# AlexGr5/StereoVision

Measured on AMD Instinct MI355X. Metric: disparity frames/sec + HBM GB/s, 1920x1080 D=128 win=9, 1/2/4/8 GPU, higher is better.
Workload: dtype u8

## Files before the change

### stereovision_amd/csrc/sv_match.hip

```cpp
#include "sv_internal.h"
#include "sv_xcd.h"

#include <algorithm>
#include <cstdlib>
#include <vector>
#include <cstdio>
#include <type_traits>

namespace sv {
namespace {

constexpr int COST_SAD4 = 4;

__host__ __device__ __forceinline__ int seg_width(int lpg, int dpl, int sm = 4) { return (sm * lpg + dpl - 1) / dpl * dpl; }
__host__ __device__ __forceinline__ int wave_cols(int lpg, int dpl, int sm = 4) { return (64 / lpg) * seg_width(lpg, dpl, sm); }
int seg_mult(int kind, int r) {
    static const int sm4 = [] {
        const char* e = std::getenv("SV_SAD4_SEG");
        const int v = e ? std::atoi(e) : 0;
        return v >= 1 && v <= 8 ? v : 0;
    }();
    if (kind != COST_SAD4) return 4;
    if (sm4) return sm4;
    return (2 * r - 2 + 3) / 4 <= 2 ? 4 : 2;
// ... 133 lines not shown
            }
#pragma unroll
            for (int q = 0; q < 4; ++q) {
                const int pos = j <= 2 ? j - q : (j >= 2 * r + 1 ? (3 - q) + (j - 2 * r - 1) : -1);
                const bool in = j <= 2 ? (j >= q) : (j >= 2 * r + 1 && j <= 2 * r + q);
                w[NC + q] |= in ? v << (8 * pos) : 0u;
            }
        }
        put<COST, ND>(dst, w);
    } else {
        uint32_t w[5] = {0u, 0u, 0u, 0u, 0u};
        uint32_t sq = 0;
        for (int j = 0; j < a.win; ++j) {
            const int yy = clampi(y - a.r + j, 0, a.H - 1);
            const uint32_t v = img[(size_t)yy * a.pitch + cc];
            sq += v * v;
            const uint32_t sh = v << (8 * (j & 3));
            const int q = j >> 2;
            w[0] |= q == 0 ? sh : 0u;
            w[1] |= q == 1 ? sh : 0u;
            w[2] |= q == 2 ? sh : 0u;
            w[3] |= q == 3 ? sh : 0u;
        }
        if constexpr (COST == COST_SSD) w[ND] = sq;
        const uint32_t o[8] = {w[0], w[1], w[2], w[3], w[4], 0u, 0u, 0u};
        put<COST, ND>(dst, o);
    }
}

__device__ __forceinline__ void transpose4(uint32_t a, uint32_t b, uint32_t c, uint32_t d, uint32_t (&o)[4]) {
    const uint32_t t0 = __builtin_amdgcn_perm(b, a, 0x05010400u);
    const uint32_t t1 = __builtin_amdgcn_perm(b, a, 0x07030602u);
    const uint32_t t2 = __builtin_amdgcn_perm(d, c, 0x05010400u);
    const uint32_t t3 = __builtin_amdgcn_perm(d, c, 0x07030602u);
    o[0] = __builtin_amdgcn_perm(t2, t0, 0x05040100u);
    o[1] = __builtin_amdgcn_perm(t2, t0, 0x07060302u);
    o[2] = __builtin_amdgcn_perm(t3, t1, 0x05040100u);
    o[3] = __builtin_amdgcn_perm(t3, t1, 0x07060302u);
}

template <int R>
__device__ __forceinline__ void sad4_group_words(const uint32_t (&rw)[2 * R + 4],
                                                 uint32_t (&w)[PackCfg<COST_SAD4, R>::NW][4]) {
    constexpr int NC = PackCfg<COST_SAD4, R>::NW - 4, NCR = 2 * R - 2;
#pragma unroll
    for (int m = 0; m < NC; ++m) {
        uint32_t d[4];
#pragma unroll
        for (int t = 0; t < 4; ++t) d[t] = 4 * m + t < NCR ? rw[3 + 4 * m + t] : 0u;
        transpose4(d[0], d[1], d[2], d[3], w[m]);
    }
#pragma unroll
    for (int q = 0; q < 4; ++q) {
        uint32_t d[3];
        int n = 0;
#pragma unroll
        for (int j = q; j <= 2; ++j) d[n++] = rw[j];
#pragma unroll
        for (int j = 2 * R + 1; j <= 2 * R + q; ++j) d[n++] = rw[j];
        transpose4(d[0], d[1], d[2], 0u, w[NC + q]);
    }
}

template <int COST, int ND>
__device__ __forceinline__ void build_group(const MatchParams& a, const uint8_t* img, int cg, int y,
                                            uint32_t (&w)[PackCfg<COST, ND>::NW][4]) {
    const int r = COST == COST_SAD4 ? ND : a.r;
    auto row = [&](int j) -> uint32_t {
        const int yy = clampi(y - r + j, 0, a.H - 1);
        return *reinterpret_cast<const uint32_t*>(img + (size_t)yy * a.pitch + cg);
    };
    if constexpr (COST == COST_SAD4) {
        uint32_t rw[2 * ND + 4];
#pragma unroll
        for (int j = 0; j < 2 * ND + 4; ++j) rw[j] = row(j);
        sad4_group_words<ND>(rw, w);
        return;
    }
    const int nsh = a.win;
#pragma unroll
    for (int q = 0; q < ND; ++q) {
        uint32_t d[4];
#pragma unroll
        for (int t = 0; t < 4; ++t) d[t] = (4 * q + t < nsh) ? row(4 * q + t) : 0u;
        transpose4(d[0], d[1], d[2], d[3], w[q]);
    }
    if constexpr (COST == COST_SSD) {
#pragma unroll
        for (int k = 0; k < 4; ++k) {
            uint32_t sq = 0u;
#pragma unroll
            for (int q = 0; q < ND; ++q) sq = __builtin_amdgcn_udot4(w[q][k], w[q][k], sq, false);
            w[ND][k] = sq;
        }
    }
}

__device__ __forceinline__ int rslot(int i, int c0, int dpl) { return i + (i + c0) / dpl; }

template <int COST, int ND, int DPL>
__device__ __forceinline__ void build_all_packs(const MatchParams& a, int y, int cL0, int NL, int cR0,
                                                int NRlog, int c0, PackOut<COST, ND> Lp,
                                                PackOut<COST, ND> Rp, int lane) {
    constexpr int NW = PackCfg<COST, ND>::NW;
    bool aligned = ((reinterpret_cast<uintptr_t>(a.L) | reinterpret_cast<uintptr_t>(a.R) |
                     (uintptr_t)a.pitch) & 3u) == 0;
    if constexpr (COST == COST_HOG) aligned = false;
    if (!aligned) {
        for (int i = lane; i < NL; i += 64) build_pack<COST, ND>(a, a.L, a.HL, cL0 + i, y, Lp + i);
        for (int i = lane; i < NRlog; i += 64)
            build_pack<COST, ND>(a, a.R, a.HR, cR0 + i, y, Rp + rslot(i, c0, DPL));
        return;
    }
    if constexpr (COST != COST_HOG) {
    const int aL = cL0 & ~3, aR = cR0 & ~3;
    const int gL = (cL0 + NL - aL + 3) >> 2, gR = (cR0 + NRlog - aR + 3) >> 2;
    for (int gi = lane; gi < gL + gR; gi += 64) {
        const bool right = gi >= gL;
        const int cg = right ? aR + 4 * (gi - gL) : aL + 4 * gi;
        const int cfirst = right ? cR0 : cL0, n = right ? NRlog : NL;
        const uint8_t* img = right ? a.R : a.L;
        const PackOut<COST, ND> base = right ? Rp : Lp;
        if (cg >= 0 && cg + 4 <= a.W) {
            uint32_t w[NW][4];
            build_group<COST, ND>(a, img, cg, y, w);
#pragma unroll
            for (int k = 0; k < 4; ++k) {
                const int idx = cg + k - cfirst;
                if (idx < 0 || idx >= n) continue;
                uint32_t v[8];
#pragma unroll
                for (int i = 0; i < 8; ++i) v[i] = i < NW ? w[i < NW ? i : 0][k] : 0u;
                put<COST, ND>(base + (right ? rslot(idx, c0, DPL) : idx), v);
            }
        } else {
#pragma unroll
            for (int k = 0; k < 4; ++k) {
                const int idx = cg + k - cfirst;
                if (idx < 0 || idx >= n) continue;
                build_pack<COST, ND>(a, img, nullptr, cg + k, y, base + (right ? rslot(idx, c0, DPL) : idx));
            }
        }
    }
    }
}

template <int R, int MF, int DPL>
__device__ __forceinline__ void build_ring_packs(const MatchParams& a, int y, int cL0, int NL, int cR0,
                                                 int NRlog, int c0, PackOut<COST_SAD4, R> Lp,
                                                 PackOut<COST_SAD4, R> Rp, int lane) {
    constexpr int NW = PackCfg<COST_SAD4, R>::NW, NRW = 2 * R + 4;
    const bool aligned = ((reinterpret_cast<uintptr_t>(a.L) | reinterpret_cast<uintptr_t>(a.R) |
                           (uintptr_t)a.pitch) & 3u) == 0;
    if (!aligned) {
        build_all_packs<COST_SAD4, R, DPL>(a, y, cL0, NL, cR0, NRlog, c0, Lp, Rp, lane);
        return;
    }
    const int aL = cL0 & ~3, aR = cR0 & ~3;
    const int gL = (cL0 + NL - aL + 3) >> 2, gR = (cR0 + NRlog - aR + 3) >> 2;
    const int G = gL + gR;
    uint32_t roff[NRW];
#pragma unroll
    for (int j = 0; j < NRW; ++j) roff[j] = (uint32_t)clampi(y - R + j, 0, a.H - 1) * (uint32_t)a.pitch;
    for (int g0 = 0; g0 < G; g0 += 64 * MF) {
        uint32_t rw[MF][NRW];
#pragma unroll
        for (int m = 0; m < MF; ++m) {
            const int gi = g0 + lane + 64 * m;
            const bool right = gi >= gL;
            const int cg = right ? aR + 4 * (gi - gL) : aL + 4 * gi;
            const bool in = gi < G && cg >= 0 && cg + 4 <= a.W;
            const uint8_t* img = (right ? a.R : a.L) + (in ? cg : 0);
#pragma unroll
            for (int j = 0; j < NRW; ++j) rw[m][j] = *reinterpret_cast<const uint32_t*>(img + roff[j]);
        }
#pragma unroll
        for (int m = 0; m < MF; ++m) {
            const int gi = g0 + lane + 64 * m;
            if (gi >= G) continue;
            const bool right = gi >= gL;
            const int cg = right ? aR + 4 * (gi - gL) : aL + 4 * gi;
            const int cfirst = right ? cR0 : cL0, n = right ? NRlog : NL;
            const PackOut<COST_SAD4, R> base = right ? Rp : Lp;
            if (cg >= 0 && cg + 4 <= a.W) {
                uint32_t w[NW][4];
                sad4_group_words<R>(rw[m], w);
#pragma unroll
                for (int k = 0; k < 4; ++k) {
                    const int idx = cg + k - cfirst;
                    if (idx < 0 || idx >= n) continue;
                    uint32_t v[8];
#pragma unroll
                    for (int i = 0; i < 8; ++i) v[i] = i < NW ? w[i < NW ? i : 0][k] : 0u;
                    put<COST_SAD4, R>(base + (right ? rslot(idx, c0, DPL) : idx), v);
                }
            } else {
#pragma unroll
                for (int k = 0; k < 4; ++k) {
                    const int idx = cg + k - cfirst;
                    if (idx < 0 || idx >= n) continue;
                    build_pack<COST_SAD4, R>(a, right ? a.R : a.L, nullptr, cg + k, y,
                                             base + (right ? rslot(idx, c0, DPL) : idx));
                }
            }
        }
    }
}

template <int COST, int ND, int DPL>
__device__ __forceinline__ void match_chunk(
    const int cut, const int dbits, PackPtr<COST, ND> rnb, PackPtr<COST, ND> rob, PackPtr<COST, ND> lnb,
    PackPtr<COST, ND> lob,
    Pk<PackCfg<COST, ND>::NW> (&rn)[DPL], Pk<PackCfg<COST, ND>::NW> (&ro)[DPL],
    uint32_t (&h)[DPL][PackCfg<COST, ND>::ROWS], const uint32_t (&mk)[DPL],
    uint32_t (&bk)[PackCfg<COST, ND>::ROWS][DPL]) {
    constexpr int NW = PackCfg<COST, ND>::NW;
    constexpr int ROWS = PackCfg<COST, ND>::ROWS;
    constexpr bool RUN = COST != COST_HOG;
    constexpr bool HI = hi_keys(COST, ND);
#pragma unroll
    for (int u = 0; u < DPL; ++u) {
        rn[u] = ld<COST, ND>(rnb + u);
        const Pk<NW> L = ld<COST, ND>(lnb + u);
        Pk<NW> LO;
        if constexpr (RUN) {
            ro[u] = ld<COST, ND>(rob + (u + (u >= cut ? 1 : 0)));
            LO = ld<COST, ND>(lob + u);
        }
#pragma unroll
        for (int k = 0; k < DPL; ++k) {
            const int sk = (u - k + DPL) % DPL;
            if constexpr (HI) {
                constexpr int NC = PackCfg<COST, ND>::NC;
                uint32_t cn = 0u, co = 0u;
#pragma unroll
                for (int i = 0; i < NC; ++i) {
                    cn = __builtin_amdgcn_sad_hi_u8(L.w[i], rn[sk].w[i], cn);
                    co = __builtin_amdgcn_sad_hi_u8(LO.w[i], ro[sk].w[i], co);
                }
                const uint32_t nch = co - cn;
#pragma unroll
                for (int q = 0; q < ROWS; ++q) {
                    const uint32_t m = __builtin_amdgcn_sad_hi_u8(LO.w[NC + q], ro[sk].w[NC + q], nch);
                    h[k][q] = __builtin_amdgcn_sad_hi_u8(L.w[NC + q], rn[sk].w[NC + q], h[k][q]) - m;
                }
                continue;
            }
            uint32_t vn[ROWS];
            ccol<COST, ND, NW>(L, rn[sk], vn);
            if constexpr (RUN) {
                uint32_t vo[ROWS];
                ccol<COST, ND, NW>(LO, ro[sk], vo);
#pragma unroll
                for (int q = 0; q < ROWS; ++q) h[k][q] = shl_add(vn[q] - vo[q], 1 << dbits, h[k][q]);
            } else {
                h[k][0] = (vn[0] << dbits) | mk[k];
            }
        }
#pragma unroll
        for (int q = 0; q < ROWS; ++q) {
            uint32_t b = 0xFFFFFFFFu;
#pragma unroll
            for (int k = 0; k < DPL; ++k) b = min(b, h[k][q]);
            bk[q][u] = b;
        }
        __builtin_amdgcn_sched_barrier(0);
    }
}

template <int LPG, int N>
__device__ __forceinline__ void reduce_batch(uint32_t* v) {
#define SV_ROR_STEP(CTRL)                                                                     \
    _Pragma("unroll") for (int i = 0; i < N; ++i)                                             \
        v[i] = min(v[i], (uint32_t)__builtin_amdgcn_update_dpp(0u, (int)v[i], CTRL, 0xF, 0xF, false));
    SV_ROR_STEP(0x121)
    SV_ROR_STEP(0x122)
    SV_ROR_STEP(0x124)
    SV_ROR_STEP(0x128)
#undef SV_ROR_STEP
    if constexpr (LPG >= 32) {
#pragma unroll
        for (int i = 0; i < N; ++i)
            v[i] = min(v[i], (uint32_t)__builtin_amdgcn_update_dpp(-1, (int)v[i], 0x142, 0xA, 0xF, false));
    }
    if constexpr (LPG == 64) {
#pragma unroll
        for (int i = 0; i < N; ++i)
            v[i] = min(v[i], (uint32_t)__builtin_amdgcn_update_dpp(-1, (int)v[i], 0x143, 0xC, 0xF, false));
    }
}

__device__ __forceinline__ void reduce_scatter16(uint32_t (&v)[16], int l) {
#define SV_RS_STEP(HALF, BIT, CTRL)                                                            \
    {                                                                                          \
        const bool hi = (l & (BIT)) != 0;                                                      \
        _Pragma("unroll") for (int k = 0; k < (HALF); ++k) {                                   \
            const uint32_t send = hi ? v[k] : v[k + (HALF)];                                   \
            const uint32_t keep = hi ? v[k + (HALF)] : v[k];                                   \
            v[k] = min(keep, (uint32_t)__builtin_amdgcn_update_dpp(0u, (int)send, CTRL, 0xF, 0xF, false)); \
        }                                                                                      \
    }
    SV_RS_STEP(8, 8, 0x140)
    SV_RS_STEP(4, 4, 0x141)
    SV_RS_STEP(2, 2, 0x1B)
    SV_RS_STEP(1, 1, 0xB1)
#undef SV_RS_STEP
}

__device__ __forceinline__ void reduce_scatter16_bm(uint32_t (&v)[16], int l) {
#define SV_BM_PAIR(A, B, CTRL, M0, M1)                                                          \
    "v_min_u32_dpp %" #A ", %" #A ", %" #A " " CTRL " row_mask:0xf bank_mask:" M0 "\n\t"      \
    "v_min_u32_dpp %" #A ", %" #B ", %" #B " " CTRL " row_mask:0xf bank_mask:" M1 "\n\t"
    asm volatile("s_nop 1\n\t"
                 SV_BM_PAIR(0, 8, "row_mirror", "0x3", "0xc") SV_BM_PAIR(1, 9, "row_mirror", "0x3", "0xc")
                 SV_BM_PAIR(2, 10, "row_mirror", "0x3", "0xc") SV_BM_PAIR(3, 11, "row_mirror", "0x3", "0xc")
                 SV_BM_PAIR(4, 12, "row_mirror", "0x3", "0xc") SV_BM_PAIR(5, 13, "row_mirror", "0x3", "0xc")
                 SV_BM_PAIR(6, 14, "row_mirror", "0x3", "0xc") SV_BM_PAIR(7, 15, "row_mirror", "0x3", "0xc")
                 : "+v"(v[0]), "+v"(v[1]), "+v"(v[2]), "+v"(v[3]), "+v"(v[4]), "+v"(v[5]), "+v"(v[6]), "+v"(v[7])
                 : "v"(v[8]), "v"(v[9]), "v"(v[10]), "v"(v[11]), "v"(v[12]), "v"(v[13]), "v"(v[14]), "v"(v[15]));
    asm volatile("s_nop 1\n\t"
                 SV_BM_PAIR(0, 4, "row_half_mirror", "0x5", "0xa") SV_BM_PAIR(1, 5, "row_half_mirror", "0x5", "0xa")
                 SV_BM_PAIR(2, 6, "row_half_mirror", "0x5", "0xa") SV_BM_PAIR(3, 7, "row_half_mirror", "0x5", "0xa")
                 : "+v"(v[0]), "+v"(v[1]), "+v"(v[2]), "+v"(v[3])
                 : "v"(v[4]), "v"(v[5]), "v"(v[6]), "v"(v[7]));
#undef SV_BM_PAIR
#define SV_RS_STEP(HALF, BIT, CTRL)                                                            \
    {                                                                                          \
// ... 148 lines not shown
    const PackPtr<COST, ND> rn0 = Rp + rslot(iN, c0, DPL);
    const PackPtr<COST, ND> ro0 = Rp + rslot(iR0, c0, DPL);
    const PackPtr<COST, ND> ln0 = Lp + (iL0 + W2);
    const PackPtr<COST, ND> lo0 = Lp + iL0;
    const int T = (S - 1 + DPL - 1) / DPL * DPL;

    for (int t0 = 0, c = 0; t0 < T; t0 += DPL, ++c) {
        match_chunk<COST, ND, DPL>(cut, dbits, rn0 + c * (DPL + 1), ro0 + c * (DPL + 1), ln0 + t0, lo0 + t0, rn,
                                   ro, h, mk, bk);
        if constexpr (ROWS * DPL == 16 || ROWS * DPL == 32) {
            if (LPG == 16) {
#pragma unroll
                for (int half = 0; half < ROWS * DPL / 16; ++half) {
                    uint32_t v[16];
#pragma unroll
                    for (int i = 0; i < 16; ++i) v[i] = bk[(16 * half + i) / DPL][i % DPL];
                    reduce_scatter16(v, l);
                    const int q = (16 * half) / DPL + l / DPL, e = t0 + l % DPL + 1, x = xs + e;
                    if (e < S && x < a.X1 && y + q < a.row1)
                        a.out[(size_t)(y + q) * a.opitch + x] = (int16_t)(((int)(v[0] & dmask) + a.minD) * 16);
                }
                continue;
            }
        }
        if constexpr (ROWS * DPL == 8) {
            uint32_t v[8];
#pragma unroll
            for (int i = 0; i < 8; ++i) v[i] = bk[i / DPL][i % DPL];
            reduce_scatter8_bm(v, lane & 15);
            uint32_t key = v[0];
            if (LPG >= 32) {
                const auto p = __builtin_amdgcn_permlane16_swap(key, key, false, false);
                key = min(p[0], p[1]);
            }
            if (LPG == 64) {
                const auto p = __builtin_amdgcn_permlane32_swap(key, key, false, false);
                key = min(p[0], p[1]);
            }
            const int i = (l >> 1) & 7, q = i / DPL, e = t0 + i % DPL + 1, x = xs + e;
            if (l < 16 && (l & 1) == 0 && e < S && x < a.X1 && y + q < a.row1)
                a.out[(size_t)(y + q) * a.opitch + x] = (int16_t)(((int)(key & dmask) + a.minD) * 16);
            continue;
        }
        const int e = t0 + j + 1;
        const int x = xs + e;
        const bool emit = j >= 0 && j < DPL && e < S && x < a.X1;
        if (LPG == 16) reduce_batch<16, ROWS * DPL>(&bk[0][0]);
        else if (LPG == 32) reduce_batch<32, ROWS * DPL>(&bk[0][0]);
        else reduce_batch<64, ROWS * DPL>(&bk[0][0]);
#pragma unroll
        for (int q = 0; q < ROWS; ++q) {
            uint32_t v = bk[q][0];
#pragma unroll
            for (int u = 1; u < DPL; ++u) v = (j == u) ? bk[q][u] : v;
            if (emit && y + q < a.row1)
                a.out[(size_t)(y + q) * a.opitch + x] = (int16_t)(((int)(v & dmask) + a.minD) * 16);
        }
    }
}

constexpr int RG_DPL = 4;

typedef unsigned short u16x2 __attribute__((ext_vector_type(2)));
__device__ __forceinline__ uint32_t pk_add16(uint32_t a, uint32_t b) {
    return __builtin_bit_cast(uint32_t, __builtin_bit_cast(u16x2, a) + __builtin_bit_cast(u16x2, b));
}
__device__ __forceinline__ uint32_t pk_sub16(uint32_t a, uint32_t b) {
    return __builtin_bit_cast(uint32_t, __builtin_bit_cast(u16x2, a) - __builtin_bit_cast(u16x2, b));
}


typedef uint32_t lds_u32x4 __attribute__((ext_vector_type(4), may_alias));
constexpr int RING_SCRATCH_BYTES = 8 * 64 * 4;

template <int R, int LPGT, bool DEFER, bool KEYS, bool SSD = false, bool LDSMIN = false>
__global__ __launch_bounds__(64, 2) void k_match_ring(MatchParams a) {
    using P = PackCfg<COST_SAD4, R>;
    constexpr int NW = P::NW, NC = P::NC, W2 = 2 * R + 1;
    static_assert(!LDSMIN || (LPGT == 32 && R <= 5), "the LDS fold is laid out for two 32-lane groups of 32-bit keys");
    constexpr bool PK = R >= 6;
    static_assert(P::SPLIT && (P::CW == 3) == PK, "ring kind expects split packs (20 B for r 2..3, 24 B for r 4..5, 28 B for r 6..7)");
    extern __shared__ __attribute__((aligned(16))) uint4 smem[];
    int bx, by, bz;
    xcd_tile(a.xcd_map != 0, bx, by, bz);
    if (bz) {
        a.L += bz * a.fs_in;
        a.R += bz * a.fs_in;
        a.out += bz * a.fs_out;
        if constexpr (KEYS) a.keys += bz * a.fs_out;
    }
    const int lane = threadIdx.x;
    constexpr int LPG = LPGT;
    const int S = a.segm;
    const int WC = (64 / LPG) * S;
    constexpr bool SADU = PK || R <= 5;
    constexpr int M = SADU ? W2 + 1 : W2;
    constexpr int U = M % 4 == 0 ? M : M % 2 == 0 ? 2 * M : 4 * M;
    constexpr int NCH = U / 4;
    const int Tn = (S + 2 * R + 3) & ~3;
    const int nit = (Tn + U - 1) / U;
    const int e0 = (nit * U - Tn) >> 2;
    const int NL = WC - S + Tn + 1;
    const int NRlog = WC - S + Tn + 4 * LPG;
    constexpr int c0 = 1;
    const int NRphys = NRlog + (NRlog + c0) / RG_DPL + 1;
    uint4* wbase = smem + (LDSMIN ? RING_SCRATCH_BYTES / 16 : 0);
    typename P::CT* cbase = reinterpret_cast<typename P::CT*>(wbase + (size_t)(NL + NRphys));
    const PackOut<COST_SAD4, R> Lw{wbase, cbase};
    const PackOut<COST_SAD4, R> Rw{wbase + NL, cbase + NL};
    const PackPtr<COST_SAD4, R> Lp{Lw.x, Lw.c};
    const PackPtr<COST_SAD4, R> Rp{Rw.x, Rw.c};

    const int y = a.row0 + by * 4;
    const int yc = min(y, a.row1 - 1);
    const int xw = a.X0 + bx * WC;
    const int cL0 = xw - R;
    const int cR0 = cL0 - a.minD - (4 * LPG - 1);
    build_ring_packs<R, 3, RG_DPL>(a, yc, cL0, NL, cR0, NRlog, c0, Lw, Rw, lane);

    if (!KEYS && bx == 0) {
        const int16_t inv = (int16_t)((a.minD - 1) * 16);
#pragma unroll
        for (int q = 0; q < 4; ++q) {
            if (y + q >= a.row1) break;
            int16_t* orow = a.out + (size_t)(y + q) * a.opitch;
            for (int x = lane; x < a.X0; x += 64) orow[x] = inv;
            for (int x = a.X1 + lane; x < a.W; x += 64) orow[x] = inv;
        }
    }
    __syncthreads();
    if (y >= a.row1) return;

    const int g = lane / LPG;
    const int l = lane & (LPG - 1);
    const int xs = xw + g * S;
    const int dl = PK ? min(4 * l, a.D - 4) : 4 * l;
    const int iR0 = g * S + 4 * (LPG - 1) - dl + 3;
    constexpr int RQ = PK ? 2 : 4;
    uint32_t h[RG_DPL][RQ], lab[RG_DPL];
#pragma unroll
    for (int k = 0; k < RG_DPL; ++k) {
        const int idx = 4 * l + k;
        const uint32_t base = PK ? 0u : idx < a.D ? (uint32_t)idx : (SSD ? a.pad_key : 0x8000u << 16) | (uint32_t)idx;
        lab[k] = (uint32_t)idx;
#pragma unroll
        for (int q = 0; q < RQ; ++q) h[k][q] = base;
    }
    uint32_t ring[M][RG_DPL][RQ];
#pragma unroll
    for (int s = 0; s < M; ++s)
#pragma unroll
        for (int k = 0; k < RG_DPL; ++k)
#pragma unroll
            for (int q = 0; q < RQ; ++q) ring[s][k][q] = 0u;
    Pk<NW> rn[RG_DPL];
#pragma unroll
    for (int s = 1; s < RG_DPL; ++s) rn[RG_DPL - s] = ld<COST_SAD4, R, true>(Rp + rslot(iR0 - s, c0, RG_DPL));
    PackPtr<COST_SAD4, R> rb = Rp + (rslot(iR0, c0, RG_DPL) - e0 * (RG_DPL + 1));
    PackPtr<COST_SAD4, R> lb = Lp + (g * S - 4 * e0);
    constexpr bool LPF = !(R == 5 && SADU);
    Pk<NW> Lnext = ld<COST_SAD4, R, true>(lb + 4 * e0);
    const int jq = (lane >> 2) & 3, ju = (lane >> 1) & 1;
    constexpr bool join2 = LPG >= 32;
    int pofs = 0;
    if (join2 && !LDSMIN) {
        const auto p = __builtin_amdgcn_permlane16_swap((uint32_t)lane, (uint32_t)lane + 64u, false, false);
        pofs = (max(p[0], p[1]) < 64u) ? 0 : 2;
    }
    const int eq = LDSMIN ? lane >> 4 : jq;
    const int exs = LDSMIN ? xw + ((lane >> 2) & 1) * S : xs;
    const int eb = (LDSMIN ? ((lane >> 3) & 1) + 2 * (lane & 1) : ju + pofs) - 2 * R;
    constexpr int OB = KEYS ? 4 : 2;
    const int ooff = OB * ((y + eq) * a.opitch + exs + eb);
    const auto orsrc = KEYS ? __builtin_amdgcn_make_buffer_rsrc(a.keys, 0, 0x7FFFFFFF, 0x00020000)
                            : __builtin_amdgcn_make_buffer_rsrc(a.out, 0, 0x7FFFFFFF, 0x00020000);
    const int emax = (LDSMIN ? (lane & 2) == 0 && y + eq < a.row1
                             : (l & 1) == 0 && l < (join2 ? 32 : 16) && y + jq < a.row1)
                         ? max(0, min(S, a.X1 - exs)) : 0;

    auto emit_key = [&](uint32_t key, int tt) {
        const int off = (unsigned)(tt + eb) < (unsigned)emax ? ooff + OB * tt : (int)0x80000000u;
        if constexpr (KEYS) __builtin_amdgcn_raw_buffer_store_b32(key, orsrc, off, 0, 0);
        else __builtin_amdgcn_raw_buffer_store_b16(
            (uint16_t)(((int)(key & (SSD ? (1u << a.dbits) - 1u : 0xFFFFu)) + a.minD) * 16), orsrc, off, 0, 0);
    };
    auto join_pairs = [&](uint32_t kA_, uint32_t kB_) {
        auto p = __builtin_amdgcn_permlane16_swap(kA_, kB_, false, false);
        uint32_t key = min(p[0], p[1]);
        if (LPG == 64) {
            p = __builtin_amdgcn_permlane32_swap(key, key, false, false);
            key = min(p[0], p[1]);
        }
        return key;
    };
    auto join_rows = [&](uint32_t key) {
        if (LPG >= 32) {
            const auto p = __builtin_amdgcn_permlane16_swap(key, key, false, false);
            key = min(p[0], p[1]);
        }
        if (LPG == 64) {
            const auto p = __builtin_amdgcn_permlane32_swap(key, key, false, false);
            key = min(p[0], p[1]);
        }
        return key;
    };
    uint32_t dv[8], kA = 0xFFFFFFFFu;
    int tprev = -(1 << 24);
#pragma unroll
    for (int i = 0; i < 8; ++i) dv[i] = 0xFFFFFFFFu;
    [[maybe_unused]] uint32_t* const scr = reinterpret_cast<uint32_t*>(smem);
    [[maybe_unused]] const uint32_t scr_m0 = __builtin_amdgcn_readfirstlane(
        (uint32_t)(uintptr_t)(__attribute__((address_space(3))) uint32_t*)scr);
    [[maybe_unused]] const lds_u32x4* const sra = reinterpret_cast<const lds_u32x4*>(scr + 8 * lane + 4 * ((lane >> 3) & 1));
    [[maybe_unused]] const lds_u32x4* const srb = reinterpret_cast<const lds_u32x4*>(scr + 8 * lane + 4 * (1 - ((lane >> 3) & 1)));
    auto lds_fold = [&](const lds_u32x4& p, const lds_u32x4& s) {
        uint32_t m = min(min(p.x, p.y), p.z);
        m = min(min(m, p.w), s.x);
        m = min(min(m, s.y), s.z);
        m = min(m, s.w);
        m = min(m, (uint32_t)__builtin_amdgcn_update_dpp(0u, (int)m, 0xB1, 0xF, 0xF, false));
        return min(m, (uint32_t)__builtin_amdgcn_update_dpp(0u, (int)m, 0x4E, 0xF, 0xF, false));
    };
    [[maybe_unused]] const bool pairB = (lane & 1) != 0;

    for (int it = 0, t0 = -4 * e0; it < nit; ++it) {
#pragma unroll
        for (int ch = 0; ch < NCH; ++ch, t0 += 4) {
            if (t0 < 0) continue;
            uint32_t bk[4][2];
#pragma unroll
            for (int u = 0; u < 4; ++u) {
                const int slot = (4 * ch + u) % M, oslot = (4 * ch + u + 1) % M;
                rn[u] = ld<COST_SAD4, R, true>(rb + (ch * (RG_DPL + 1) + u));
                const Pk<NW> Lc = LPF ? Lnext : ld<COST_SAD4, R, true>(lb + (4 * ch + u));
                if constexpr (LPF) Lnext = ld<COST_SAD4, R, true>(lb + (4 * ch + u + 1));
                lds_u32x4 fa{}, fb{};
                if constexpr (LDSMIN) {
                    if ((u & 1) == 0) { fa = *sra; fb = *srb; }
                }
                uint32_t sqL[4];
                if constexpr (SSD) {
                    uint32_t sc = 0u;
#pragma unroll
                    for (int i = 0; i < NC; ++i) sc = __builtin_amdgcn_udot4(Lc.w[i], Lc.w[i], sc, false);
#pragma unroll
                    for (int q = 0; q < 4; ++q)
                        sqL[q] = __builtin_amdgcn_udot4(Lc.w[NC + q], Lc.w[NC + q], sc, false) << a.dbits;
                }
                if constexpr (!SADU) {
#pragma unroll
                    for (int k = 0; k < RG_DPL; ++k)
#pragma unroll
                        for (int q = 0; q < RQ; ++q)
                            h[k][q] = PK ? pk_sub16(h[k][q], ring[slot][k][q]) : h[k][q] - ring[slot][k][q];
                }
#pragma unroll
                for (int kk = 0; kk < RG_DPL; ++kk) {
                    const int k = RG_DPL - 1 - kk;
                    const Pk<NW>& Rk = rn[(u - k) & 3];
                    if constexpr (PK) {
                        uint32_t cn = 0u;
#pragma unroll
                        for (int i = 0; i < NC; ++i) cn = __builtin_amdgcn_sad_u8(Lc.w[i], Rk.w[i], cn);
                        cn |= cn << 16;
#pragma unroll
                        for (int j = 0; j < 2; ++j) {
                            const uint32_t c = __builtin_amdgcn_sad_hi_u8(
                                Lc.w[NC + 2 * j + 1], Rk.w[NC + 2 * j + 1],
                                __builtin_amdgcn_sad_u8(Lc.w[NC + 2 * j], Rk.w[NC + 2 * j], cn));
                            if constexpr (SADU) sad_u32_acc(h[k][j], ring[oslot][k][j], c);
                            else h[k][j] = pk_add16(h[k][j], c);
                            ring[slot][k][j] = c;
                        }
                    } else if constexpr (SSD) {
                        uint32_t cn = 0u, sr = 0u;
#pragma unroll
                        for (int i = 0; i < NC; ++i) {
                            cn = __builtin_amdgcn_udot4(Lc.w[i], Rk.w[i], cn, false);
                            sr = __builtin_amdgcn_udot4(Rk.w[i], Rk.w[i], sr, false);
                        }
#pragma unroll
                        for (int q = 0; q < 4; ++q) {
                            const uint32_t lr = __builtin_amdgcn_udot4(Lc.w[NC + q], Rk.w[NC + q], cn, false);
                            const uint32_t rr = __builtin_amdgcn_udot4(Rk.w[NC + q], Rk.w[NC + q], sr, false);
                            const uint32_t t = (rr << a.dbits) + sqL[q];
                            const uint32_t c = (uint32_t)__mul24((int)lr, -(2 << a.dbits)) + t;
                            sad_u32_acc(h[k][q], ring[oslot][k][q], c);
                            ring[slot][k][q] = c;
                        }
                    } else {
                        uint32_t cn = 0u;
#pragma unroll
                        for (int i = 0; i < NC; ++i) cn = __builtin_amdgcn_sad_hi_u8(Lc.w[i], Rk.w[i], cn);
#pragma unroll
                        for (int q = 0; q < 4; ++q) {
                            const uint32_t c = __builtin_amdgcn_sad_hi_u8(Lc.w[NC + q], Rk.w[NC + q], cn);
                            if constexpr (SADU) sad_u32_acc(h[k][q], ring[oslot][k][q], c);
                            else h[k][q] += c;
                            ring[slot][k][q] = c;
                        }
                    }
                }
#pragma unroll
                for (int q = 0; q < 4; ++q) {
                    uint32_t kq[RG_DPL];
#pragma unroll
                    for (int k = 0; k < RG_DPL; ++k)
                        kq[k] = !PK ? h[k][q] : (q & 1) ? (h[k][q >> 1] & 0xFFFF0000u) | lab[k] : (h[k][q >> 1] << 16) | lab[k];
                    bk[q][u & 1] = min(min(kq[0], kq[1]), min(kq[2], kq[3]));
                }
                if constexpr (LDSMIN) {
                    if (u == 2) {
                        kA = lds_fold(fa, fb);
                    } else if (u == 0) {
                        const uint32_t kB = lds_fold(fa, fb);
                        emit_key(pairB ? kB : kA, tprev);
                        tprev = t0;
                    }
                }
                __builtin_amdgcn_sched_barrier(0);
                if constexpr (LDSMIN) {
                    if (u & 1) {
                        asm volatile("s_mov_b32 m0, %8\n\t"
                                     "s_nop 0\n\t"
                                     "ds_write_addtid_b32 %0\n\t"
                                     "ds_write_addtid_b32 %1 offset:256\n\t"
                                     "ds_write_addtid_b32 %2 offset:512\n\t"
                                     "ds_write_addtid_b32 %3 offset:768\n\t"
                                     "ds_write_addtid_b32 %4 offset:1024\n\t"
                                     "ds_write_addtid_b32 %5 offset:1280\n\t"
                                     "ds_write_addtid_b32 %6 offset:1536\n\t"
                                     "ds_write_addtid_b32 %7 offset:1792\n\t"
                                     :
                                     : "v"(bk[0][0]), "v"(bk[0][1]), "v"(bk[1][0]), "v"(bk[1][1]), "v"(bk[2][0]),
                                       "v"(bk[2][1]), "v"(bk[3][0]), "v"(bk[3][1]), "s"(scr_m0)
                                     : "memory", "m0");
                        __builtin_amdgcn_fence(__ATOMIC_SEQ_CST, "wavefront");
                    }
                    continue;
                }
                if (DEFER && u == 3) {
#pragma unroll
                    for (int i = 0; i < 8; ++i) dv[i] = bk[i >> 1][i & 1];
                } else if (DEFER && u == 1) {
                    uint32_t v[8];
#pragma unroll
                    for (int i = 0; i < 8; ++i) v[i] = bk[i >> 1][i & 1];
                    reduce_scatter8_bm(v, lane & 15);
                    reduce_scatter8_bm(dv, lane & 15);
                    if (join2) {
                        emit_key(join_pairs(kA, dv[0]), tprev);
                        kA = v[0];
                    } else {
                        emit_key(join_rows(dv[0]), tprev + 2);
                        emit_key(join_rows(v[0]), t0);
                    }
                    tprev = t0;
                } else if (u & 1) {
                    uint32_t v[8];
#pragma unroll
                    for (int i = 0; i < 8; ++i) v[i] = bk[i >> 1][i & 1];
                    reduce_scatter8_bm(v, lane & 15);
                    if (join2) {
                        if (u == 1) kA = v[0];
                        else emit_key(join_pairs(kA, v[0]), t0);
                    } else {
                        emit_key(join_rows(v[0]), t0 + u - 1);
                    }
                }
            }
        }
        rb = rb + NCH * (RG_DPL + 1);
        lb = lb + U;
    }
    if constexpr (LDSMIN) {
        const uint32_t kB = lds_fold(*sra, *srb);
        emit_key(pairB ? kB : kA, tprev);
    } else if (DEFER) {
        reduce_scatter8_bm(dv, lane & 15);
        if (join2) emit_key(join_pairs(kA, dv[0]), tprev);
        else emit_key(join_rows(dv[0]), tprev + 2);
    }
}

__global__ void k_fill_i16(int16_t* out, int opitch, int H, int W, int16_t v) {
    const int x = blockIdx.x * blockDim.x + threadIdx.x;
    const int y = blockIdx.y;
    if (x < W && y < H) out[(size_t)y * opitch + x] = v;
}

template <int COST, int ND, int DPL>
int launch_one(const MatchParams& a, size_t lds, hipStream_t s) {
    auto fn = k_match<COST, ND, DPL>;
    if (lds > 65536) {
        hipError_t e = hipFuncSetAttribute((const void*)fn, hipFuncAttributeMaxDynamicSharedMemorySize, (int)lds);
        if (e != hipSuccess) return (int)e;
    }
    const int wc = wave_cols(a.lpg, DPL, a.segm);
    const int rows_per_block = PackCfg<COST, ND>::WPB * PackCfg<COST, ND>::ROWS;
    dim3 grid((a.X1 - a.X0 + wc - 1) / wc, (a.row1 - a.row0 + rows_per_block - 1) / rows_per_block,
              a.nf > 1 ? a.nf : 1);
    hipLaunchKernelGGL(fn, grid, dim3(64 * PackCfg<COST, ND>::WPB), lds, s, a);
    return (int)hipGetLastError();
}

template <int COST, int ND>
int launch_dpl(const MatchParams& a, const MatchPlan& p, size_t lds, hipStream_t s) {
    switch (p.dpl) {
        case 4: return launch_one<COST, ND, 4>(a, lds, s);
        case 6: return launch_one<COST, ND, 6>(a, lds, s);
        case 8: return launch_one<COST, ND, 8>(a, lds, s);
    }
    return (int)hipErrorInvalidValue;
}

template <int COST>
int launch_nd(const MatchParams& a, const MatchPlan& p, size_t lds, hipStream_t s) {
    if constexpr (COST == COST_HOG) {
        return launch_dpl<COST, 5>(a, p, lds, s);
    } else if constexpr (COST == COST_SAD4) {
        switch (p.ndw) {
            case 2: return launch_dpl<COST, 2>(a, p, lds, s);
            case 3: return launch_dpl<COST, 3>(a, p, lds, s);
            case 4: return launch_dpl<COST, 4>(a, p, lds, s);
            case 5: return launch_dpl<COST, 5>(a, p, lds, s);
            case 6: return launch_dpl<COST, 6>(a, p, lds, s);
            case 7: return launch_dpl<COST, 7>(a, p, lds, s);
        }
        return (int)hipErrorInvalidValue;
    } else {
        switch (p.ndw) {
            case 1: return launch_dpl<COST, 1>(a, p, lds, s);
            case 2: return launch_dpl<COST, 2>(a, p, lds, s);
            case 3: return launch_dpl<COST, 3>(a, p, lds, s);
            case 4: return launch_dpl<COST, 4>(a, p, lds, s);
        }
        return (int)hipErrorInvalidValue;
    }
}

int kind_of(int cost, int win) {
    if (cost == COST_SAD && win >= 5) return COST_SAD4;
    return cost;
}

bool ring_kind(int cost, int win, int num_disp) {
    static const bool on = [] {
        const char* e = std::getenv("SV_RING");
        return !(e && e[0] == '0');
    }();
    return on && kind_of(cost, win) == COST_SAD4 && win >= 5 && num_disp <= 256 &&
           (win <= 11 || (win <= 15 && num_disp % 4 == 0));
}
int ring_lpg(int num_disp) { return num_disp <= 64 ? 16 : num_disp <= 128 ? 32 : 64; }
bool ring_ldsmin(int lpg, int r, bool keys, bool ssd) {
    static const bool on = [] {
        const char* e = std::getenv("SV_RING_LDSMIN");
        return !(e && e[0] == '0');
    }();
    return on && lpg == 32 && r == 4 && !keys && !ssd;
}
size_t ring_lds_bytes(int lpg, int seg, int r, bool ldsmin);
int ring_seg(int lpg, int r, int band, long long blocks, bool ldsmin) {
    static const int env = [] {
        const char* e = std::getenv("SV_RING_SEG");
        const int v = e ? std::atoi(e) : 0;
        return v >= 8 && v <= 1024 && v % 4 == 0 ? v : 0;
    }();
    (void)blocks;
    if (env) return env;
    const int G = 64 / lpg;
    int best = 8;
    long long best_cost = -1;
    for (int S = 8; S <= 1024; S += 4) {
        if (S > 8 && ring_lds_bytes(lpg, S, r, ldsmin) > 20 * 1024) break;
        const long long cost = (long long)((band + G * S - 1) / (G * S)) * ((S + 2 * r + 3) & ~3);
        if (best_cost < 0 || cost <= best_cost) { best = S; best_cost = cost; }
    }
    return best;
}
size_t ring_lds_bytes(int lpg, int seg, int r, bool ldsmin) {
    const int wc = (64 / lpg) * seg;
    const int tn = (seg + 2 * r + 3) & ~3;
    const int nl = wc - seg + tn + 1, nr = wc - seg + tn + 4 * lpg;
    const int nrp = nr + (nr + 1) / RG_DPL + 1;
    return (size_t)(nl + nrp) * (r <= 3 ? 20 : r <= 5 ? 24 : 28) + (ldsmin ? RING_SCRATCH_BYTES : 0);
}

template <int R, int LPG, bool KEYS, bool SSD>
int launch_ring_rl(const MatchParams& a, size_t lds, hipStream_t s) {
    static const bool defer = [] {
        const char* e = std::getenv("SV_RING_DEFER");
        return !(e && e[0] == '0');
    }();
    void (*fn)(MatchParams);
    if constexpr (SSD) fn = k_match_ring<R, LPG, R != 5, false, true>;
    else if constexpr (KEYS) fn = k_match_ring<R, LPG, R != 5, true>;
    else fn = (defer && R != 5) ? k_match_ring<R, LPG, R != 5, false> : k_match_ring<R, LPG, false, false>;
    if constexpr (R == 4 && LPG == 32 && !KEYS && !SSD) {
        if (ring_ldsmin(LPG, R, KEYS, SSD)) fn = k_match_ring<R, LPG, false, false, false, true>;
    }
    if (lds > 65536) {
        hipError_t e = hipFuncSetAttribute((const void*)fn, hipFuncAttributeMaxDynamicSharedMemorySize, (int)lds);
        if (e != hipSuccess) return (int)e;
    }
    const int wc = (64 / a.lpg) * a.segm;
    dim3 grid((a.X1 - a.X0 + wc - 1) / wc, (a.row1 - a.row0 + 3) / 4, a.nf > 1 ? a.nf : 1);
    static const bool occ = [] {
        const char* e = std::getenv("SV_RING_OCC");
        return e && e[0] == '1';
    }();
    if (occ) {
        int nb = -1;
        (void)hipOccupancyMaxActiveBlocksPerMultiprocessor(&nb, (const void*)fn, 64, lds);
        std::fprintf(stderr, "k_match_ring r=%d lpg=%d ldsmin=%d seg=%d lds=%zu B: %d waves/CU\n", R, LPG,
                     (int)ring_ldsmin(LPG, R, KEYS, SSD), a.segm, lds, nb);
    }
    static const bool xcd = [] {
        const char* e = std::getenv("SV_XCD_MAP");
        return !(e && e[0] == '0');
    }();
    MatchParams b = a;
    b.xcd_map = xcd ? 1 : 0;
// ... 191 lines not shown
```

Before: 31040.

## Peel SAD warm-up chunks and use buffer loads for ring pack building

```diff
diff --git a/stereovision_amd/csrc/sv_match.hip b/stereovision_amd/csrc/sv_match.hip
--- a/stereovision_amd/csrc/sv_match.hip
+++ b/stereovision_amd/csrc/sv_match.hip
@@ -309,16 +309,19 @@
     constexpr int NW = PackCfg<COST_SAD4, R>::NW, NRW = 2 * R + 4;
     const bool aligned = ((reinterpret_cast<uintptr_t>(a.L) | reinterpret_cast<uintptr_t>(a.R) |
                            (uintptr_t)a.pitch) & 3u) == 0;
-    if (!aligned) {
+    const bool near = (long long)a.H * (long long)a.pitch < 0x7FFFFFFFLL;
+    if (!aligned || !near) {
         build_all_packs<COST_SAD4, R, DPL>(a, y, cL0, NL, cR0, NRlog, c0, Lp, Rp, lane);
         return;
     }
+    const auto lsrc = __builtin_amdgcn_make_buffer_rsrc(const_cast<uint8_t*>(a.L), 0, 0x7FFFFFFF, 0x00020000);
+    const auto rsrc = __builtin_amdgcn_make_buffer_rsrc(const_cast<uint8_t*>(a.R), 0, 0x7FFFFFFF, 0x00020000);
     const int aL = cL0 & ~3, aR = cR0 & ~3;
     const int gL = (cL0 + NL - aL + 3) >> 2, gR = (cR0 + NRlog - aR + 3) >> 2;
     const int G = gL + gR;
-    uint32_t roff[NRW];
-#pragma unroll
-    for (int j = 0; j < NRW; ++j) roff[j] = (uint32_t)clampi(y - R + j, 0, a.H - 1) * (uint32_t)a.pitch;
+    int roff[NRW];
+#pragma unroll
+    for (int j = 0; j < NRW; ++j) roff[j] = clampi(y - R + j, 0, a.H - 1) * a.pitch;
     for (int g0 = 0; g0 < G; g0 += 64 * MF) {
         uint32_t rw[MF][NRW];
 #pragma unroll
@@ -327,9 +330,14 @@
             const bool right = gi >= gL;
             const int cg = right ? aR + 4 * (gi - gL) : aL + 4 * gi;
             const bool in = gi < G && cg >= 0 && cg + 4 <= a.W;
-            const uint8_t* img = (right ? a.R : a.L) + (in ? cg : 0);
-#pragma unroll
-            for (int j = 0; j < NRW; ++j) rw[m][j] = *reinterpret_cast<const uint32_t*>(img + roff[j]);
+            if (in && !right) {
+#pragma unroll
+                for (int j = 0; j < NRW; ++j) rw[m][j] = __builtin_amdgcn_raw_buffer_load_b32(lsrc, cg, roff[j], 0);
+            }
+            if (in && right) {
+#pragma unroll
+                for (int j = 0; j < NRW; ++j) rw[m][j] = __builtin_amdgcn_raw_buffer_load_b32(rsrc, cg, roff[j], 0);
+            }
         }
 #pragma unroll
         for (int m = 0; m < MF; ++m) {
@@ -784,7 +792,7 @@
 #pragma unroll
         for (int k = 0; k < RG_DPL; ++k)
 #pragma unroll
-            for (int q = 0; q < RQ; ++q) ring[s][k][q] = 0u;
+            for (int q = 0; q < RQ; ++q) asm volatile("" : "=v"(ring[s][k][q]));
     Pk<NW> rn[RG_DPL];
 #pragma unroll
     for (int s = 1; s < RG_DPL; ++s) rn[RG_DPL - s] = ld<COST_SAD4, R, true>(Rp + rslot(iR0 - s, c0, RG_DPL));
@@ -855,11 +863,10 @@
     };
     [[maybe_unused]] const bool pairB = (lane & 1) != 0;
 
-    for (int it = 0, t0 = -4 * e0; it < nit; ++it) {
-#pragma unroll
-        for (int ch = 0; ch < NCH; ++ch, t0 += 4) {
-            if (t0 < 0) continue;
-            uint32_t bk[4][2];
+    constexpr int NZ = 2 * R - 4 * (2 * R / 4) + 1;
+    auto chunk = [&](auto warm_c, const int ch, const int t0) __attribute__((always_inline)) {
+            constexpr bool WARM = decltype(warm_c)::value;
+            [[maybe_unused]] uint32_t bk[4][2];
 #pragma unroll
             for (int u = 0; u < 4; ++u) {
                 const int slot = (4 * ch + u) % M, oslot = (4 * ch + u + 1) % M;
@@ -867,7 +874,7 @@
                 const Pk<NW> Lc = LPF ? Lnext : ld<COST_SAD4, R, true>(lb + (4 * ch + u));
                 if constexpr (LPF) Lnext = ld<COST_SAD4, R, true>(lb + (4 * ch + u + 1));
                 lds_u32x4 fa{}, fb{};
-                if constexpr (LDSMIN) {
+                if constexpr (LDSMIN && !WARM) {
                     if ((u & 1) == 0) { fa = *sra; fb = *srb; }
                 }
                 uint32_t sqL[4];
@@ -879,7 +886,7 @@
                     for (int q = 0; q < 4; ++q)
                         sqL[q] = __builtin_amdgcn_udot4(Lc.w[NC + q], Lc.w[NC + q], sc, false) << a.dbits;
                 }
-                if constexpr (!SADU) {
+                if constexpr (!SADU && !WARM) {
 #pragma unroll
                     for (int k = 0; k < RG_DPL; ++k)
 #pragma unroll
@@ -900,7 +907,7 @@
                             const uint32_t c = __builtin_amdgcn_sad_hi_u8(
                                 Lc.w[NC + 2 * j + 1], Rk.w[NC + 2 * j + 1],
                                 __builtin_amdgcn_sad_u8(Lc.w[NC + 2 * j], Rk.w[NC + 2 * j], cn));
-                            if constexpr (SADU) sad_u32_acc(h[k][j], ring[oslot][k][j], c);
+                            if constexpr (SADU && !WARM) sad_u32_acc(h[k][j], ring[oslot][k][j], c);
                             else h[k][j] = pk_add16(h[k][j], c);
                             ring[slot][k][j] = c;
                         }
@@ -917,7 +924,8 @@
                             const uint32_t rr = __builtin_amdgcn_udot4(Rk.w[NC + q], Rk.w[NC + q], sr, false);
                             const uint32_t t = (rr << a.dbits) + sqL[q];
                             const uint32_t c = (uint32_t)__mul24((int)lr, -(2 << a.dbits)) + t;
-                            sad_u32_acc(h[k][q], ring[oslot][k][q], c);
+                            if constexpr (WARM) h[k][q] += c;
+                            else sad_u32_acc(h[k][q], ring[oslot][k][q], c);
                             ring[slot][k][q] = c;
                         }
                     } else {
@@ -927,11 +935,15 @@
 #pragma unroll
                         for (int q = 0; q < 4; ++q) {
                             const uint32_t c = __builtin_amdgcn_sad_hi_u8(Lc.w[NC + q], Rk.w[NC + q], cn);
-                            if constexpr (SADU) sad_u32_acc(h[k][q], ring[oslot][k][q], c);
+                            if constexpr (SADU && !WARM) sad_u32_acc(h[k][q], ring[oslot][k][q], c);
                             else h[k][q] += c;
                             ring[slot][k][q] = c;
                         }
                     }
+                }
+                if constexpr (WARM) {
+                    __builtin_amdgcn_sched_barrier(0);
+                    continue;
                 }
 #pragma unroll
                 for (int q = 0; q < 4; ++q) {
@@ -1001,6 +1013,29 @@
                     }
                 }
             }
+            if constexpr (WARM) {
+                if (t0 + 7 >= 2 * R) {
+#pragma unroll
+                    for (int i = 0; i < NZ; ++i)
+#pragma unroll
+                        for (int k = 0; k < RG_DPL; ++k)
+#pragma unroll
+                            for (int q = 0; q < RQ; ++q) ring[(4 * ch + 5 + i) % M][k][q] = 0u;
+                }
+            }
+    };
+    constexpr int NWARM = 2 * R / 4;
+#pragma unroll
+    for (int e = 0; e < NCH; ++e) {
+        if (e != e0) continue;
+#pragma unroll
+        for (int i = 0; i < NWARM; ++i) chunk(std::true_type{}, e + i, 4 * i);
+    }
+    for (int it = 0, t0 = -4 * e0; it < nit; ++it) {
+#pragma unroll
+        for (int ch = 0; ch < NCH; ++ch, t0 += 4) {
+            if (t0 < 4 * NWARM) continue;
+            chunk(std::false_type{}, ch, t0);
         }
         rb = rb + NCH * (RG_DPL + 1);
         lb = lb + U;
```

After: 31890, median of 6. 2.8% higher.
